# VealFang/PLI-SLAM

Hardware: AMD Instinct MI355X
Metric: stereo frames/sec (ORB+LSD extract+match), 752x480 EuRoC (higher is better)
Workload: dtype u8; 1 GPU; 1xMI355X: 752x480 stereo pairs, extract + stereo Hamming match (BASELINE configs[1] shape, batched); 752x480, 1200 ORB kp (8 levels x1.2) + LSD/LBD (<=100 lines); 256 stereo frames per GPU per step; frames_per_gpu=256, parallelism=frame-batch data parallel, 1 rank(s), gather of result tables to rank 0

## Files before the change

### pli_slam_amd/csrc/kernels.hpp

```cpp
#pragma once
#include "common.hpp"

namespace pli {

struct BlurPlane {
  int w, h, pitchIn, pitchOut;
  int64_t offIn, offOut;
  int tilesX, tileBase;
};
struct BlurJob {
  int nplanes;
  BlurPlane pl[MAX_LEVELS];
  int k[7];
  int radius;
};
struct LbdCoef { float L[21]; float G[63]; };
constexpr int PROJ_K = 64;
__global__ void k_ingest_copy16(const uint8_t* __restrict__ left, const uint8_t* __restrict__ right, int64_t stride, int64_t frameStride, uint8_t* __restrict__ pyr, int64_t pyrBlock, int W16, int H, int pitch, int img0);
__global__ void k_ingest(const uint8_t* __restrict__ left, const uint8_t* __restrict__ right, int64_t stride, int64_t frameStride, uint8_t* __restrict__ pyr, int64_t pyrBlock, int W, int H, int pitch, const float2* __restrict__ mapL, const float2* __restrict__ mapR, int img0);
__global__ void k_resize_level(const uint8_t* __restrict__ srcBase, int64_t srcImgStride, int sw, int sh, int spitch, uint8_t* __restrict__ dstBase, int64_t dstImgStride, int dw, int dh, int dpitch, const int* __restrict__ tab, int img0);
__global__ void k_fast_cells(const DevParams* __restrict__ Pp, const uint8_t* __restrict__ pyr, uint32_t* __restrict__ cellCand, int* __restrict__ cellCount, int img0);
__global__ void k_octree(const DevParams* __restrict__ Pp, const uint32_t* __restrict__ cellCand, const int* __restrict__ cellCount, uint32_t* __restrict__ candAll, unsigned short* __restrict__ nodeOfAll, int* __restrict__ candCount, uint32_t* __restrict__ kpSel, int* __restrict__ kpSelCount, int img0);
__global__ void k_octree_512(const DevParams* __restrict__ Pp, const uint32_t* __restrict__ cellCand, const int* __restrict__ cellCount, uint32_t* __restrict__ candAll, unsigned short* __restrict__ nodeOfAll, int* __restrict__ candCount, uint32_t* __restrict__ kpSel, int* __restrict__ kpSelCount, int img0);
__global__ void k_octree_320(const DevParams* __restrict__ Pp, const uint32_t* __restrict__ cellCand, const int* __restrict__ cellCount, uint32_t* __restrict__ candAll, unsigned short* __restrict__ nodeOfAll, int* __restrict__ candCount, uint32_t* __restrict__ kpSel, int* __restrict__ kpSelCount, int img0);
__global__ void k_octree_w(const DevParams* __restrict__ Pp, const uint32_t* __restrict__ cellCand, const int* __restrict__ cellCount, uint32_t* __restrict__ candAll, unsigned short* __restrict__ nodeOfAll, int* __restrict__ candCount, uint32_t* __restrict__ kpSel, int* __restrict__ kpSelCount, int img0);
__global__ void k_octree_512_w(const DevParams* __restrict__ Pp, const uint32_t* __restrict__ cellCand, const int* __restrict__ cellCount, uint32_t* __restrict__ candAll, unsigned short* __restrict__ nodeOfAll, int* __restrict__ candCount, uint32_t* __restrict__ kpSel, int* __restrict__ kpSelCount, int img0);
__global__ void k_octree_320_w(const DevParams* __restrict__ Pp, const uint32_t* __restrict__ cellCand, const int* __restrict__ cellCount, uint32_t* __restrict__ candAll, unsigned short* __restrict__ nodeOfAll, int* __restrict__ candCount, uint32_t* __restrict__ kpSel, int* __restrict__ kpSelCount, int img0);
__global__ void k_blur(const BlurJob* __restrict__ Jp, const uint8_t* __restrict__ in, int64_t inImgStride, uint8_t* __restrict__ out, int64_t outImgStride, int img0);
__global__ void k_describe(const DevParams* __restrict__ Pp, const uint8_t* __restrict__ pyr, const uint8_t* __restrict__ blur, const uint32_t* __restrict__ kpSel, const int* __restrict__ kpSelCount, uint8_t* __restrict__ table, int64_t recordBytes, int64_t offCounts, int64_t offKp0, int64_t offKp1, int64_t offDesc0, int64_t offDesc1, int img0);
__global__ void k_kp_counts(const DevParams* __restrict__ Pp, const int* __restrict__ kpSelCount, uint8_t* __restrict__ table, int64_t recordBytes, int64_t offCounts, int nimg, int img0);
__global__ void k_lsd_grad(const uint8_t* __restrict__ scaled, int64_t imgStride, int W, int H, int WP, int pitch, int g2Thresh, float4* __restrict__ rec, int* __restrict__ g2o, int2* __restrict__ own, int* __restrict__ maxG2, float* __restrict__ angDbg, int img0, int trigF32);
__global__ void k_lsd_hist(const int* __restrict__ g2a, int npix, int g2Thresh, int nBins, const int* __restrict__ maxG2, unsigned short* __restrict__ chunkHist, int nChunks, int img0, const double* __restrict__ mgAll, const unsigned long long* __restrict__ maxMg, double rho, const RxCtl* __restrict__ onlyUnsettled);
__global__ void k_lsd_scan(const unsigned short* __restrict__ chunkHist, int nChunks, int nBins, int* __restrict__ chunkBase, int* __restrict__ nDefined, int img0, const RxCtl* __restrict__ onlyUnsettled);
__global__ void k_lsd_scatter(const int* __restrict__ g2a, int npix, int g2Thresh, int nBins, const int* __restrict__ maxG2, const int* __restrict__ chunkBase, int nChunks, int* __restrict__ order, int img0, int nimg, const double* __restrict__ mgAll, const unsigned long long* __restrict__ maxMg, double rho, int* __restrict__ rankAll, const int* __restrict__ groupOff, int chunksPerGroup, int nGroups, const RxCtl* __restrict__ onlyUnsettled);
__global__ void k_lsd_scan_part(const unsigned short* __restrict__ chunkHist, int nChunks, int nBins, int chunksPerGroup, int* __restrict__ chunkBase, int* __restrict__ groupOff, int img0, const RxCtl* __restrict__ onlyUnsettled);
__global__ void k_lsd_scan_groups(int nGroups, int nBins, int* __restrict__ groupOff, int* __restrict__ nDefined, int img0, const RxCtl* __restrict__ onlyUnsettled);
__global__ void k_lsd_grow_unsettled(const DevParams* __restrict__ Pp, float4* __restrict__ recAll, const double* __restrict__ mgAll, const int* __restrict__ orderAll, const int* __restrict__ nDefined, uint2* __restrict__ regOverflow, float* __restrict__ segAll, int* __restrict__ nSeg, int maxSeg, int img0, int nimg, RxCtl* __restrict__ ctl);
__global__ void k_lsd_grow(const DevParams* __restrict__ Pp, float4* __restrict__ recAll, const double* __restrict__ mgAll, const int* __restrict__ orderAll, const int* __restrict__ nDefined, uint2* __restrict__ regOverflow, float* __restrict__ segAll, int* __restrict__ nSeg, int maxSeg, int img0, int nimg);
__global__ void k_lsd_grow2(const DevParams* __restrict__ Pp, float4* __restrict__ recAll, const double* __restrict__ mgAll, const int* __restrict__ orderAll, const int* __restrict__ nDefined, uint2* __restrict__ regOverflow, float* __restrict__ segAll, int* __restrict__ nSeg, int maxSeg, int img0, int nimg);
__global__ void k_lsd_grow_spec(const DevParams* __restrict__ Pp, float4* __restrict__ recAll, const double* __restrict__ mgAll, const int* __restrict__ orderAll, const int* __restrict__ nDefined, uint2* __restrict__ regOverflow, float* __restrict__ segAll, int* __restrict__ nSeg, int maxSeg, int img0, int nimg, LsdRectItem* __restrict__ rectAll, double* __restrict__ rectWAll);
__global__ void k_lsd_grow2_spec(const DevParams* __restrict__ Pp, float4* __restrict__ recAll, const double* __restrict__ mgAll, const int* __restrict__ orderAll, const int* __restrict__ nDefined, uint2* __restrict__ regOverflow, float* __restrict__ segAll, int* __restrict__ nSeg, int maxSeg, int img0, int nimg, LsdRectItem* __restrict__ rectAll, double* __restrict__ rectWAll);
__global__ void k_lsd_rect(const DevParams* __restrict__ Pp, const LsdRectItem* __restrict__ rectAll, const uint2* __restrict__ arenaAll, const double* __restrict__ mgAll, const double* __restrict__ rectWAll, const int* __restrict__ nSeg, float* __restrict__ segAll, int maxSeg, int img0);
__global__ void k_keylines(const DevParams* __restrict__ Pp, const float* __restrict__ seg, const int* __restrict__ nSeg, int maxSeg, pli_keyline* __restrict__ tmpKL, uint8_t* __restrict__ table, int64_t recordBytes, int64_t offCounts, int64_t offKl0, int64_t offKl1, int img0);
__global__ void k_sobel(const uint8_t* __restrict__ in, int64_t imgStride, int W, int H, int pitch, short2* __restrict__ dxy, int img0);
__global__ void k_lbd(const DevParams* __restrict__ Pp, const LbdCoef* __restrict__ coef, const short2* __restrict__ dxya, uint8_t* __restrict__ table, int64_t recordBytes, int64_t offCounts, int64_t offKl0, int64_t offKl1, int64_t offLd0, int64_t offLd1, float* __restrict__ dbgFloat, int img0);
__global__ void k_lsd_blur64(const uint8_t* __restrict__ pyr, int64_t pyrBlock, int W, int H, int pitch, const double* __restrict__ kern, int radius, double* __restrict__ out, int64_t outImgStride, int img0);
__global__ void k_lsd_resize64(const double* __restrict__ src, int sw, int sh, double* __restrict__ dst, int dw, int dh, int64_t dstImgStride, const int* __restrict__ tab, int img0);
__global__ void k_lsd_grad64(const double* __restrict__ scaled, int W, int H, int WP, int64_t scaledImgStride, double rho, float4* __restrict__ rec, double* __restrict__ mg, int2* __restrict__ own, unsigned long long* __restrict__ maxMg, float* __restrict__ angDbg, int img0, int flags, int2* __restrict__ hot, float2* __restrict__ cold);
__global__ void k_lsd_front64(const uint8_t* __restrict__ pyr, int64_t pyrBlock, int sw, int sh, int pitch, const double* __restrict__ kern, int radius, const int* __restrict__ tab, int dw, int dh, int dp, double rho, float4* __restrict__ rec, double* __restrict__ mg, int2* __restrict__ own, unsigned long long* __restrict__ maxMg, int img0, int flags, int2* __restrict__ hot, float2* __restrict__ cold);
__global__ void k_rx_guess(const float4* __restrict__ recAll, const int* __restrict__ rankAll, int2* __restrict__ ownAll, int W, int H, float precDeg, int img0);
__global__ void k_rx_diff(RxCtl* __restrict__ ctl, const int2* __restrict__ ownAll, int* __restrict__ tileMinAll, int* __restrict__ tileActAll, int W, int H, int TW, int TH, int t, int img0, const int* __restrict__ tileTouchAll);
__global__ void k_rx_classify(RxCtl* __restrict__ ctl, const int2* __restrict__ ownAll, const int* __restrict__ rankAll, const int2* __restrict__ rgBoxAll, uint8_t* __restrict__ rgCleanAll, const int* __restrict__ tileMinAll, int W, int H, int TW, int TH, int t, int img0);
__global__ void k_rx_seed(RxCtl* __restrict__ ctl, int2* __restrict__ ownAll, const int* __restrict__ rankAll, const float4* __restrict__ recAll, const int* __restrict__ rgSizeAll, const uint8_t* __restrict__ rgCleanAll, RxSeed* __restrict__ smallAll, RxSeed* __restrict__ bigAll, int bigCap, int W, int H, int bigThresh, int t, int img0);
__global__ void k_rx_mark(RxCtl* __restrict__ ctl, const int2* __restrict__ ownAll, const int* __restrict__ rankAll, const int2* __restrict__ rgBoxAll, int* __restrict__ rgDirtyAll, const int* __restrict__ tileMinAll, int* __restrict__ tileActAll, int W, int H, int TW, int TH, int t, int img0, int seedRule, const int* __restrict__ rgLostAll, TxDirtyLists DL);
__global__ void k_rx_seed_sparse(RxCtl* __restrict__ ctl, int2* __restrict__ ownAll, const int* __restrict__ rankAll, const float4* __restrict__ recAll, const int* __restrict__ rgSizeAll, const int* __restrict__ rgDirtyAll, const int* __restrict__ tileActAll, RxSeed* __restrict__ smallAll, RxSeed* __restrict__ bigAll, int bigCap, int W, int H, int TW, int TH, int bigThresh, int t, int img0);
__global__ void k_rx_grow(const DevParams* __restrict__ Pp, RxCtl* __restrict__ ctl, const float4* __restrict__ recAll, int2* __restrict__ ownAll, const RxSeed* __restrict__ smallAll, int* __restrict__ rgSizeAll, int2* __restrict__ rgBoxAll, RxHand* __restrict__ handAll, int handCap, int* __restrict__ arenaAll, int arenaCap, RxRect* __restrict__ rectAll, int rectCap, int img0, int t);
__global__ void k_rx_grow_big(const DevParams* __restrict__ Pp, RxCtl* __restrict__ ctl, const float4* __restrict__ recAll, int2* __restrict__ ownAll, const RxSeed* __restrict__ bigAll, int bigCap, const RxHand* __restrict__ handAll, int handCap, int* __restrict__ rgSizeAll, int2* __restrict__ rgBoxAll, int* __restrict__ arenaAll, int arenaCap, RxRect* __restrict__ rectAll, int rectCap, int img0, int t);
__global__ void k_rx_grow_wave(const DevParams* __restrict__ Pp, RxCtl* __restrict__ ctl, const float4* __restrict__ recAll, int2* __restrict__ ownAll, const RxSeed* __restrict__ bigAll, int bigCap, const RxHand* __restrict__ handAll, int handCap, int* __restrict__ rgSizeAll, int2* __restrict__ rgBoxAll, int* __restrict__ arenaAll, int arenaCap, RxRect* __restrict__ rectAll, int rectCap, int img0, int t);
__global__ void k_rx_rect(const DevParams* __restrict__ Pp, RxCtl* __restrict__ ctl, const float4* __restrict__ recAll, const int* __restrict__ arenaAll, int arenaCap, const RxRect* __restrict__ rectAll, int rectCap, float4* __restrict__ rgSegAll, int img0, const double* __restrict__ mgAll, int rmask, const int2* __restrict__ hotAll, const float2* __restrict__ coldAll);
// ... 60 lines not shown
```

### pli_slam_amd/csrc/line_kernels.hip

```cpp
#include "kernels.hpp"
#include "device_prims.hpp"
#include <type_traits>

namespace pli {

constexpr float LSD_NOTDEF = -1024.f;
constexpr double D_PI = 3.14159265358979323846;
constexpr double D_DEG2RAD = D_PI / 180;
constexpr double D_3_2_PI = (3 * D_PI) / 2;
constexpr double D_2PI = 2 * D_PI;

constexpr int LSD_GRAD_ROWS = 16;

__global__ __launch_bounds__(256) void k_lsd_grad(const uint8_t* __restrict__ scaled, int64_t imgStride, int W, int H,
                                                  int WP ,
                                                  int pitch, int g2Thresh, float4* __restrict__ rec,
                                                  int* __restrict__ g2o, int2* __restrict__ own,
                                                  int* __restrict__ maxG2, float* __restrict__ angDbg, int img0, int trigF32) {
  __shared__ int wmax[4];
  const int img = blockIdx.z + img0;
  const int x = blockIdx.x * 256 + threadIdx.x;
  int m = 0;
  if (x < WP) {
    const int yEnd = min((int)(blockIdx.y + 1) * LSD_GRAD_ROWS, H);
// ... 1329 lines not shown
      }
      if (i < M && rank < nf) {
        pli_keyline kl = tk[i];
        kl.class_id = rank;
        out[rank] = kl;
      }
    }
    if (tid == 0) reinterpret_cast<int*>(rec + offCounts)[2 + eye] = nf;
  } else {
    const int cnt = min(M, P.klCap);
    for (int i = tid; i < cnt; i += 256) out[i] = tk[i];
    if (tid == 0) reinterpret_cast<int*>(rec + offCounts)[2 + eye] = cnt;
  }
}

__global__ __launch_bounds__(256) void k_sobel(const uint8_t* __restrict__ in, int64_t imgStride, int W, int H,
                                               int pitch, short2* __restrict__ dxy, int img0) {
  const int img = blockIdx.z + img0, y = blockIdx.y, x0 = (blockIdx.x * 256 + threadIdx.x) * 4;
  const int lane = threadIdx.x & 63;
  const uint8_t* base = in + (int64_t)img * imgStride;
  const uint8_t* rows[3] = {base + (int64_t)reflect101(y - 1, H) * pitch, base + (int64_t)y * pitch, base + (int64_t)reflect101(y + 1, H) * pitch};
  const bool live = x0 < W;
  int v[3][6];
#pragma unroll
  for (int r = 0; r < 3; ++r) {
    unsigned cur = 0u;
    if (live) cur = *reinterpret_cast<const unsigned*>(rows[r] + x0);
    unsigned prev = (unsigned)__shfl_up((int)cur, 1, 64), next = (unsigned)__shfl_down((int)cur, 1, 64);
    if (lane == 0 && live && x0 >= 4) prev = *reinterpret_cast<const unsigned*>(rows[r] + x0 - 4);
    if (lane == 63 && x0 + 4 < W) next = *reinterpret_cast<const unsigned*>(rows[r] + x0 + 4);
    v[r][1] = cur & 0xFF; v[r][2] = (cur >> 8) & 0xFF; v[r][3] = (cur >> 16) & 0xFF; v[r][4] = cur >> 24;
    v[r][0] = x0 == 0 ? v[r][2] : (int)(prev >> 24);
    v[r][5] = (int)(next & 0xFF);
  }
  if (!live) return;
  if (x0 + 4 >= W) {
#pragma unroll
    for (int r = 0; r < 3; ++r)
#pragma unroll
      for (int k = 1; k < 6; ++k)
        if (x0 + k - 1 >= W) v[r][k] = rows[r][reflect101(min(x0 + k - 1, W), W)];
  }
  short2 o[4];
#pragma unroll
  for (int k = 0; k < 4; ++k) {
    const int gx = (v[0][k + 2] - v[0][k]) + 2 * (v[1][k + 2] - v[1][k]) + (v[2][k + 2] - v[2][k]);
    const int gy = (v[2][k] - v[0][k]) + 2 * (v[2][k + 1] - v[0][k + 1]) + (v[2][k + 2] - v[0][k + 2]);
    o[k] = make_short2((short)gx, (short)gy);
  }
  short2* dst = dxy + (int64_t)img * W * H + (int64_t)y * W + x0;
  if (x0 + 3 < W && (((int64_t)y * W + x0) & 3) == 0 && ((int64_t)W * H & 3) == 0) {
    *reinterpret_cast<int4*>(dst) = make_int4(*reinterpret_cast<int*>(&o[0]), *reinterpret_cast<int*>(&o[1]),
                                              *reinterpret_cast<int*>(&o[2]), *reinterpret_cast<int*>(&o[3]));
  } else {
    for (int k = 0; k < 4 && x0 + k < W; ++k) dst[k] = o[k];
  }
}

__constant__ int c_lbd_comb[32][2] = {
    {0, 1}, {0, 2}, {0, 3}, {0, 4}, {0, 5}, {0, 6}, {1, 2}, {1, 3}, {1, 4}, {1, 5}, {1, 6},
    {2, 3}, {2, 4}, {2, 5}, {2, 6}, {2, 7}, {2, 8}, {3, 4}, {3, 5}, {3, 6}, {3, 7}, {3, 8},
    {4, 5}, {4, 6}, {4, 7}, {4, 8}, {5, 6}, {5, 7}, {5, 8}, {6, 7}, {6, 8}, {7, 8}};


__global__ __launch_bounds__(64) void k_lbd(const DevParams* __restrict__ Pp, const LbdCoef* __restrict__ coef,
                                            const short2* __restrict__ dxya,
                                            uint8_t* __restrict__ table, int64_t recordBytes, int64_t offCounts,
                                            int64_t offKl0, int64_t offKl1, int64_t offLd0, int64_t offLd1,
                                            float* __restrict__ dbgFloat, int img0) {
  __shared__ float rowS[63][4];
// ... 118 lines not shown
```

### pli_slam_amd/csrc/orb_kernels.hip

```cpp
#include "kernels.hpp"
#include <type_traits>
#include "device_prims.hpp"

namespace pli {

__constant__ signed char c_orb_pattern[1024] = {
#include "../../include/pli_orb_pattern.inc"
};

__global__ __launch_bounds__(256) void k_ingest_copy16(const uint8_t* __restrict__ left, const uint8_t* __restrict__ right, int64_t stride,
                                                       int64_t frameStride, uint8_t* __restrict__ pyr, int64_t pyrBlock, int W16, int H,
                                                       int pitch, int img0) {
  const int img = blockIdx.y + img0;
  const uint8_t* src = ((img & 1) ? right : left) + (int64_t)(img >> 1) * frameStride;
  uint8_t* dst = pyr + (int64_t)img * pyrBlock;
  const int n = W16 * H;
  for (int i = blockIdx.x * 256 + threadIdx.x; i < n; i += gridDim.x * 256) {
    const int y = i / W16, x = (i - y * W16) * 16;
    *reinterpret_cast<uint4*>(dst + (int64_t)y * pitch + x) = *reinterpret_cast<const uint4*>(src + (int64_t)y * stride + x);
  }
}

__global__ __launch_bounds__(256) void k_ingest(const uint8_t* __restrict__ left, const uint8_t* __restrict__ right,
                                                int64_t stride, int64_t frameStride, uint8_t* __restrict__ pyr,
// ... 688 lines not shown
        s[0] += kc[k] * v.x; s[1] += kc[k] * v.y; s[2] += kc[k] * v.z; s[3] += kc[k] * v.w;
      }
      uint8_t o[4];
#pragma unroll
      for (int i = 0; i < 4; ++i) {
        int v = (s[i] + (1 << 15)) >> 16;
        o[i] = (uint8_t)(v < 0 ? 0 : (v > 255 ? 255 : v));
      }
      uint8_t* d = dst + (int64_t)(y0 + y) * PL.pitchOut + x0 + 4 * j;
      if (x0 + 4 * j + 3 < PL.w) *reinterpret_cast<uchar4*>(d) = make_uchar4(o[0], o[1], o[2], o[3]);
      else for (int i = 0; i < 4 && x0 + 4 * j + i < PL.w; ++i) d[i] = o[i];
    }
  }
}

__global__ __launch_bounds__(64) void k_describe(const DevParams* __restrict__ Pp, const uint8_t* __restrict__ pyr,
                                                 const uint8_t* __restrict__ blur, const uint32_t* __restrict__ kpSel,
                                                 const int* __restrict__ kpSelCount, uint8_t* __restrict__ table,
                                                 int64_t recordBytes, int64_t offCounts, int64_t offKp0,
                                                 int64_t offKp1, int64_t offDesc0, int64_t offDesc1, int img0) {
  const DevParams& P = *Pp;
  const int img = blockIdx.y + img0, slot = blockIdx.x;
  int lvl = 0;
#pragma unroll 1
  for (int l = 1; l < P.nlevels; ++l)
    if (slot >= P.lv[l].kpBase) lvl = l;
  const LevelGeom& G = P.lv[lvl];
  const int p = slot - G.kpBase;
  const int* cnts = kpSelCount + img * P.nlevels;
  if (p >= cnts[lvl]) return;
  int before = 0, total = 0;
  for (int l = 0; l < P.nlevels; ++l) {
    int c = cnts[l];
    if (l < lvl) before += c;
    total += c;
  }
  const int lane = threadIdx.x;
  uint8_t* rec = table + (int64_t)(img >> 1) * recordBytes;
  const int eye = img & 1;
  (void)offCounts; (void)total;
  const int outIdx = before + p;
  if (outIdx >= P.kpCap) return;
  const uint32_t cv = kpSel[(int64_t)img * P.kpSlotsPerImage + slot];
  const int kx = (int)((cv >> 8) & 0xFFF) + G.minBX, ky = (int)(cv >> 20) + G.minBY;
  const int resp = (int)(cv & 0xFF);
  const uint8_t* im = pyr + (int64_t)img * P.pyrBlock + G.offset;
  __shared__ int s_umax[16];
  if (lane < 16) s_umax[lane] = P.umax[lane];
  __syncthreads();
  int m10 = 0, m01 = 0;
  int val[16];
#pragma unroll
  for (int k = 0; k < 16; ++k) {
    const int i = lane + 64 * k;
    const int r = (i * 2115) >> 16;
    const int v = r - 15, u = (i - r * 31) - 15;
    const int av = v < 0 ? -v : v, au = u < 0 ? -u : u;
    val[k] = 0;
    if (i < 31 * 31 && au <= s_umax[av]) val[k] = im[(int64_t)(ky + v) * G.pitch + kx + u];
  }
#pragma unroll
  for (int k = 0; k < 16; ++k) {
    const int i = lane + 64 * k;
    const int r = (i * 2115) >> 16;
    m10 += ((i - r * 31) - 15) * val[k];
    m01 += (r - 15) * val[k];
  }
  m10 = wave_sum_i32(m10);
  m01 = wave_sum_i32(m01);
  const float angle = fast_atan2_deg((float)m01, (float)m10);
  const float factorPI = (float)(3.14159265358979323846 / 180.f);
  const float ang = __fmul_rn(angle, factorPI);
  float a, b;
  sincos_of_float(ang, (P.parityFlags & PLI_PARITY_TRIG_F32_ORB) != 0, &b, &a);
  const uint8_t* bl = blur + (int64_t)img * P.pyrBlock + G.offset;
  const uint8_t* center = bl + (int64_t)ky * G.pitch + kx;
  unsigned long long words[4];
#pragma unroll
  for (int j = 0; j < 4; ++j) {
    const signed char* pt = c_orb_pattern + 4 * (64 * j + lane);
    float x0 = (float)pt[0], y0 = (float)pt[1], x1 = (float)pt[2], y1 = (float)pt[3];
    int r0 = cv_round_f(__fadd_rn(__fmul_rn(x0, b), __fmul_rn(y0, a)));
    int c0 = cv_round_f(__fsub_rn(__fmul_rn(x0, a), __fmul_rn(y0, b)));
    int r1 = cv_round_f(__fadd_rn(__fmul_rn(x1, b), __fmul_rn(y1, a)));
    int c1 = cv_round_f(__fsub_rn(__fmul_rn(x1, a), __fmul_rn(y1, b)));
    int t0 = center[(int64_t)r0 * G.pitch + c0];
    int t1 = center[(int64_t)r1 * G.pitch + c1];
    words[j] = __ballot(t0 < t1);
  }
  if (lane == 0) {
    pli_keypoint kp;
    kp.x = (float)kx; kp.y = (float)ky;
    if (lvl != 0) { kp.x = __fmul_rn((float)kx, G.scale); kp.y = __fmul_rn((float)ky, G.scale); }
    kp.size = (float)(int)__fmul_rn(31.f, G.scale);
    kp.angle = angle;
    kp.response = (float)resp;
    kp.octave = lvl;
    reinterpret_cast<pli_keypoint*>(rec + (eye ? offKp1 : offKp0))[outIdx] = kp;
    unsigned long long* d = reinterpret_cast<unsigned long long*>(rec + (eye ? offDesc1 : offDesc0) + (int64_t)outIdx * 32);
    d[0] = words[0]; d[1] = words[1]; d[2] = words[2]; d[3] = words[3];
  }
}
// ... 32 lines not shown
```

### pli_slam_amd/csrc/pli_capi.hip

```cpp
#include "kernels.hpp"
#include "scratch_plan.hpp"
#include <cmath>
#include <cfloat>
#include <algorithm>
#include <memory>
#include <limits>
#include <cstdlib>
#include <set>
#include <string>
#include <functional>
#include <mutex>
#include <atomic>
#include <dlfcn.h>

using namespace pli;

#ifdef PLI_DEV
#define DEVENV(name) getenv(name)
#else
static inline const char* pli_no_devenv() { return nullptr; }
#define DEVENV(name) (pli_no_devenv())
#endif

namespace {
// ... 409 lines not shown
  L.off_ldesc[0] = take((int64_t)lc * 32);
  L.off_ldesc[1] = take((int64_t)lc * 32);
  L.off_disp = take((int64_t)lc * 8);
  L.off_le = take((int64_t)lc * 24);
  L.record_bytes = alignUp(o, 256);
}

pli_status allocAll(pli_ctx* c) {
  const DevParams& P = c->hp;
  const int NI = c->NI;
  pli_status st;
#define A(ptr, n) if ((st = c->dalloc(&(ptr), (size_t)(n))) != PLI_OK) return st
  A(c->dP, 1);
  HIPCHK(hipMemcpy(c->dP, &c->hp, sizeof(DevParams), hipMemcpyHostToDevice));
  A(c->pyr, (size_t)P.pyrBlock * NI);
  A(c->blur, (size_t)P.pyrBlock * NI);
  for (int l = 1; l < P.nlevels; ++l) {
    const LevelGeom &S = P.lv[l - 1], &D = P.lv[l];
    std::vector<int> t = buildResizeTab(S.w, S.h, D.w, D.h, 1. / ((double)D.w / S.w), 1. / ((double)D.h / S.h));
    A(c->resizeTab[l], t.size());
    HIPCHK(hipMemcpy(c->resizeTab[l], t.data(), t.size() * 4, hipMemcpyHostToDevice));
  }
  A(c->cellCand, (size_t)NI * P.cellsPerImage * CELL_CAP);
  A(c->cellCount, (size_t)NI * P.cellsPerImage);
  A(c->candAll, (size_t)NI * P.candPerImage);
  A(c->nodeOf, (size_t)NI * P.candPerImage);
  A(c->candCount, (size_t)NI * P.nlevels);
  A(c->kpSel, (size_t)NI * P.kpSlotsPerImage);
  A(c->kpSelCount, (size_t)NI * P.nlevels);
  {
    BlurJob J;
    std::memset(&J, 0, sizeof(J));
    J.nplanes = P.nlevels;
    J.radius = 3;
    gaussKernelFixed8(7, 2.0, J.k);
    int tb = 0;
    for (int l = 0; l < P.nlevels; ++l) {
      BlurPlane& p = J.pl[l];
      p.w = P.lv[l].w; p.h = P.lv[l].h; p.pitchIn = p.pitchOut = P.lv[l].pitch;
      p.offIn = p.offOut = P.lv[l].offset;
      p.tilesX = (p.w + 63) / 64;
      p.tileBase = tb;
      tb += p.tilesX * ((p.h + 31) / 32);
    }
    c->orbTiles = tb;
    A(c->jobOrb, 1);
    HIPCHK(hipMemcpy(c->jobOrb, &J, sizeof(J), hipMemcpyHostToDevice));
    c->tmpPitch = (int)alignUp(P.W, 64);
    c->tmp8Stride = alignUp((int64_t)c->tmpPitch * P.H, 256);
    std::memset(&J, 0, sizeof(J));
    J.nplanes = 1;
    const double sigma = (c->cfg.lsd_scale < 1) ? (c->cfg.lsd_sigma_scale / c->cfg.lsd_scale) : c->cfg.lsd_sigma_scale;
    const unsigned h = (unsigned)std::ceil(sigma * std::sqrt(2 * 3.0 * std::log(10.0)));
    if (h > 3) { g_err = "LSD pre-filter radius > 3 not supported"; return PLI_ERR_INVALID; }
    J.radius = (int)h;
    gaussKernelFixed8(1 + 2 * (int)h, sigma, J.k);
    J.pl[0].w = P.W; J.pl[0].h = P.H; J.pl[0].pitchIn = P.lv[0].pitch; J.pl[0].pitchOut = c->tmpPitch;
    J.pl[0].offIn = P.lv[0].offset; J.pl[0].offOut = 0;
    J.pl[0].tilesX = (P.W + 63) / 64; J.pl[0].tileBase = 0;
    c->l0Tiles = J.pl[0].tilesX * ((P.H + 31) / 32);
    A(c->jobLsd, 1);
    HIPCHK(hipMemcpy(c->jobLsd, &J, sizeof(J), hipMemcpyHostToDevice));
    J.radius = 2;
    std::memset(J.k, 0, sizeof(J.k));
    gaussKernelFixed8(5, 1.0, J.k);
    A(c->jobLbd, 1);
    HIPCHK(hipMemcpy(c->jobLbd, &J, sizeof(J), hipMemcpyHostToDevice));
  }
  A(c->tmp8, (size_t)c->tmp8Stride * NI);
  c->lsdStride = alignUp((int64_t)P.lpitch * P.LH, 256);
  A(c->lsdScaled, (size_t)c->lsdStride * NI);
  if (c->cfg.lsd_scale != 1) {
    std::vector<int> t = buildResizeTab(P.W, P.H, P.LWt, P.LH, 1. / c->cfg.lsd_scale, 1. / c->cfg.lsd_scale);
    A(c->lsdTab, t.size());
    HIPCHK(hipMemcpy(c->lsdTab, t.data(), t.size() * 4, hipMemcpyHostToDevice));
  }
  const size_t npix = (size_t)P.LW * P.LH;
  A(c->rec, npix * NI);
  c->lsdF64 = (c->cfg.parity_flags & PLI_PARITY_LSD_F64) != 0;
  if (c->lsdF64) {
// ... 249 lines not shown
  }
  if (P.cellsPerImage > 0)
    LAUNCH(c, "k_fast_cells", k_fast_cells, dim3(P.cellsPerImage, nimg), dim3(256), 0, c->dP, c->pyr, c->cellCand, c->cellCount, img0);
  {
    int need = 0;
    for (int l = 0; l < P.nlevels; ++l) need = std::max(need, std::max(P.lv[l].nfeatures + 8, 4 * P.lv[l].nIni + 8));
    bool wide = P.nlevels * nimg <= 1024;
    if (const char* e = DEVENV("PLI_OCTREE_WIDE")) wide = atoi(e) != 0;
    const dim3 og(P.nlevels, nimg), ob(wide ? 1024 : 256);
#define OCTREE_LAUNCH(K) LAUNCH(c, "k_octree", K, og, ob, 0, c->dP, c->cellCand, c->cellCount, c->candAll, c->nodeOf, c->candCount, c->kpSel, c->kpSelCount, img0)
    if (need <= 320) { if (wide) OCTREE_LAUNCH(k_octree_320_w); else OCTREE_LAUNCH(k_octree_320); }
    else if (need <= 512) { if (wide) OCTREE_LAUNCH(k_octree_512_w); else OCTREE_LAUNCH(k_octree_512); }
    else { if (wide) OCTREE_LAUNCH(k_octree_w); else OCTREE_LAUNCH(k_octree); }
#undef OCTREE_LAUNCH
  }
  LAUNCH(c, "k_blur_orb", k_blur, dim3(c->orbTiles, nimg), dim3(256), 0, c->jobOrb, c->pyr, P.pyrBlock, c->blur, P.pyrBlock, img0);
  LAUNCH(c, "k_kp_counts", k_kp_counts, dim3((nimg + 63) / 64), dim3(64), 0, c->dP, c->kpSelCount, table, Y.record_bytes,
         Y.off_counts, nimg, img0);
  LAUNCH(c, "k_describe", k_describe, dim3(P.kpSlotsPerImage, nimg), dim3(64), 0, c->dP, c->pyr, c->blur, c->kpSel,
         c->kpSelCount, table, Y.record_bytes, Y.off_counts, Y.off_kp[0], Y.off_kp[1], Y.off_desc[0], Y.off_desc[1], img0);
  return PLI_OK;
}

#define TRL(c, name, ...)                                                      \
  do {                                                                         \
    LAUNCH(c, rxn(name), __VA_ARGS__);                                         \
    if (trace) {                                                               \
      HIPCHK(hipStreamSynchronize((c)->stream));                               \
      std::fprintf(stderr, "[rx] %s done\n", name);                           \
    }                                                                          \
  } while (0)

pli_status runLbdPre(pli_ctx* c, int img0, int nimg) {
  TraceRange range__("pli:lbd blur+sobel");
  const DevParams& P = c->hp;
  LAUNCH(c, "k_blur_lbd", k_blur, dim3(c->l0Tiles, nimg), dim3(256), 0, c->jobLbd, c->pyr, P.pyrBlock, c->tmp8, c->tmp8Stride, img0);
  dim3 g((P.W + 1023) / 1024, P.H, nimg);
  LAUNCH(c, "k_sobel", k_sobel, g, dim3(256), 0, c->tmp8, c->tmp8Stride, P.W, P.H, c->tmpPitch, c->dxy, img0);
  return PLI_OK;
}

pli_status runLines(pli_ctx* c, int img0, int nimg, uint8_t* table) {
  TraceRange range__("pli:line chain");
  const DevParams& P = c->hp;
  const pli_table_layout& Y = c->lay;
  const int npix = P.LW * P.LH;
  const bool sequential = c->lsdMode == 2 || (c->lsdMode == 0 && (nimg >= RX_AUTO_IMAGES || nimg > c->rxImages));
  int2* ownPlane = (sequential || c->lsdMode != 1) ? (int2*)nullptr : c->own;
  const bool lostRule0 = c->lsdMode != 1 && DEVENV("PLI_TX_BOXRULE") == nullptr;
  const bool keyMode = !sequential && c->lsdMode != 1 && c->txKeys && !c->debug && lostRule0 && !DEVENV("PLI_TX_FULL2") &&
                       !DEVENV("PLI_TX_OLDMARK") && !DEVENV("PLI_TX_CELLRULE");
  int packMode = 0;
  if (!sequential && c->lsdMode != 1 && c->lsdF64 && c->mg && lostRule0 && !c->debug && !DEVENV("PLI_TX_FULL2") && !DEVENV("PLI_TX_NOFUSE2") &&
// ... 1911 lines not shown
  for (const std::string& nme : orderNames) {
    std::snprintf(line, sizeof(line), "%s %d %.6f\n", nme.c_str(), acc[nme].first, acc[nme].second);
    s += line;
  }
  if ((int64_t)s.size() + 1 > bytes) { g_err = "report buffer too small"; return PLI_ERR_CAPACITY; }
  std::memcpy(buf, s.c_str(), s.size() + 1);
  return PLI_OK;
}

pli_status pli_debug_enable(pli_ctx* c, int32_t on) {
  CtxGuard guard__(c);
  if (!c) return PLI_ERR_INVALID;
  HIPCHK(hipStreamSynchronize(c->stream));
  if (on && !c->angDbg) {
    pli_status st;
    if ((st = c->dalloc(&c->angDbg, (size_t)c->hp.LW * c->hp.LH * c->NI)) != PLI_OK) return st;
    if ((st = c->dalloc(&c->lbdFloat, (size_t)c->NI * c->hp.klCap * 72)) != PLI_OK) return st;
    if (c->lsdF64 && (st = c->dalloc(&c->scaled64Dbg, (size_t)c->hp.LW * c->hp.LH * c->NI)) != PLI_OK) return st;
  }
  c->debug = on != 0;
  return PLI_OK;
}

pli_status pli_debug_fetch(pli_ctx* c, int32_t image, int32_t what, int32_t arg, void* dst, int64_t dstBytes, int64_t* outBytes) {
  CtxGuard guard__(c);
  if (!c || image < 0 || image >= c->NI || !outBytes) { g_err = "bad argument"; return PLI_ERR_INVALID; }
  HIPCHK(hipSetDevice(c->device));
  HIPCHK(hipStreamSynchronize(c->stream));
  const DevParams& P = c->hp;
  auto need = [&](int64_t n) -> bool { *outBytes = n; return dst && dstBytes >= n; };
  switch (what) {
    case PLI_DBG_PYRAMID_LEVEL:
    case PLI_DBG_BLUR_LEVEL: {
      if (arg < 0 || arg >= P.nlevels) return PLI_ERR_INVALID;
      const LevelGeom& G = P.lv[arg];
      if (!need((int64_t)G.w * G.h)) return dst ? PLI_ERR_CAPACITY : PLI_OK;
      const uint8_t* base = (what == PLI_DBG_PYRAMID_LEVEL ? c->pyr : c->blur) + (int64_t)image * P.pyrBlock + G.offset;
      HIPCHK(hipMemcpy2D(dst, G.w, base, G.pitch, G.w, G.h, hipMemcpyDeviceToHost));
      return PLI_OK;
    }
    case PLI_DBG_FAST_CANDIDATES:
    case PLI_DBG_LEVEL_KEYPOINTS: {
      if (arg < 0 || arg >= P.nlevels) return PLI_ERR_INVALID;
      const LevelGeom& G = P.lv[arg];
      int n = 0;
      const int* cntp = (what == PLI_DBG_FAST_CANDIDATES ? c->candCount : c->kpSelCount) + image * P.nlevels + arg;
      HIPCHK(hipMemcpy(&n, cntp, 4, hipMemcpyDeviceToHost));
      if (!need(4 + (int64_t)n * 12)) return dst ? PLI_ERR_CAPACITY : PLI_OK;
      std::vector<uint32_t> raw(std::max(n, 1));
      const uint32_t* src = what == PLI_DBG_FAST_CANDIDATES ? c->candAll + (int64_t)image * P.candPerImage + G.candBase
// ... 96 lines not shown
    case PLI_DBG_STEREO_SAD: {
      const int frame = image >> 1;
      const int64_t n = (int64_t)P.kpCap * 4;
      if (!need(2 * n)) return dst ? PLI_ERR_CAPACITY : PLI_OK;
      HIPCHK(hipMemcpy(dst, c->sad + (int64_t)frame * P.kpCap, n, hipMemcpyDeviceToHost));
      HIPCHK(hipMemcpy((char*)dst + n, c->bestIdx + (int64_t)frame * P.kpCap, n, hipMemcpyDeviceToHost));
      return PLI_OK;
    }
    default:
      g_err = "unknown debug item";
      return PLI_ERR_INVALID;
  }
}

}
```

Baseline: 6315 stereo frames/s.

## Fuse ORB blur into describe and LBD blur into sobel via LDS tiles

k_describe now stages a window around each keypoint in LDS, blurs it locally with v_dot4 separable passes, and samples the BRIEF pattern from that tile instead of reading a full-image blurred pyramid. k_sobel likewise blurs a tile in shared memory before computing gradients, so the separate k_blur launches and the intermediate blur buffers are dropped. This removes full-image blur passes and their global memory traffic, but the blur work is repeated for overlapping keypoint windows, and each describe block now does more LDS work and syncs.

```diff
diff --git a/pli_slam_amd/csrc/kernels.hpp b/pli_slam_amd/csrc/kernels.hpp
--- a/pli_slam_amd/csrc/kernels.hpp
+++ b/pli_slam_amd/csrc/kernels.hpp
@@ -15,6 +15,24 @@
   int radius;
 };
 struct LbdCoef { float L[21]; float G[63]; };
+
+constexpr signed char ORB_PATTERN_HOST[1024] = {
+#include "../../include/pli_orb_pattern.inc"
+};
+constexpr int orbPatternReach() {
+  int best = 0;
+  for (int i = 0; i < 512; ++i) {
+    const long long x = ORB_PATTERN_HOST[2 * i], y = ORB_PATTERN_HOST[2 * i + 1], r2 = x * x + y * y;
+    int n = 0;
+    while ((long long)(2 * n + 1) * (2 * n + 1) * 10000 <= 4 * r2 * 10002) ++n;
+    best = n > best ? n : best;
+  }
+  return best;
+}
+constexpr int ORB_REACH = orbPatternReach();
+constexpr int ORB_BLUR_R = 3;
+constexpr int ORB_HALF_PATCH = 15;
+constexpr int LBD_BLUR_R = 2;
 constexpr int PROJ_K = 64;
 __global__ void k_ingest_copy16(const uint8_t* __restrict__ left, const uint8_t* __restrict__ right, int64_t stride, int64_t frameStride, uint8_t* __restrict__ pyr, int64_t pyrBlock, int W16, int H, int pitch, int img0);
 __global__ void k_ingest(const uint8_t* __restrict__ left, const uint8_t* __restrict__ right, int64_t stride, int64_t frameStride, uint8_t* __restrict__ pyr, int64_t pyrBlock, int W, int H, int pitch, const float2* __restrict__ mapL, const float2* __restrict__ mapR, int img0);
@@ -27,7 +45,7 @@
 __global__ void k_octree_512_w(const DevParams* __restrict__ Pp, const uint32_t* __restrict__ cellCand, const int* __restrict__ cellCount, uint32_t* __restrict__ candAll, unsigned short* __restrict__ nodeOfAll, int* __restrict__ candCount, uint32_t* __restrict__ kpSel, int* __restrict__ kpSelCount, int img0);
 __global__ void k_octree_320_w(const DevParams* __restrict__ Pp, const uint32_t* __restrict__ cellCand, const int* __restrict__ cellCount, uint32_t* __restrict__ candAll, unsigned short* __restrict__ nodeOfAll, int* __restrict__ candCount, uint32_t* __restrict__ kpSel, int* __restrict__ kpSelCount, int img0);
 __global__ void k_blur(const BlurJob* __restrict__ Jp, const uint8_t* __restrict__ in, int64_t inImgStride, uint8_t* __restrict__ out, int64_t outImgStride, int img0);
-__global__ void k_describe(const DevParams* __restrict__ Pp, const uint8_t* __restrict__ pyr, const uint8_t* __restrict__ blur, const uint32_t* __restrict__ kpSel, const int* __restrict__ kpSelCount, uint8_t* __restrict__ table, int64_t recordBytes, int64_t offCounts, int64_t offKp0, int64_t offKp1, int64_t offDesc0, int64_t offDesc1, int img0);
+__global__ void k_describe(const DevParams* __restrict__ Pp, const uint8_t* __restrict__ pyr, const BlurJob* __restrict__ Jp, const uint32_t* __restrict__ kpSel, const int* __restrict__ kpSelCount, uint8_t* __restrict__ table, int64_t recordBytes, int64_t offCounts, int64_t offKp0, int64_t offKp1, int64_t offDesc0, int64_t offDesc1, int img0);
 __global__ void k_kp_counts(const DevParams* __restrict__ Pp, const int* __restrict__ kpSelCount, uint8_t* __restrict__ table, int64_t recordBytes, int64_t offCounts, int nimg, int img0);
 __global__ void k_lsd_grad(const uint8_t* __restrict__ scaled, int64_t imgStride, int W, int H, int WP, int pitch, int g2Thresh, float4* __restrict__ rec, int* __restrict__ g2o, int2* __restrict__ own, int* __restrict__ maxG2, float* __restrict__ angDbg, int img0, int trigF32);
 __global__ void k_lsd_hist(const int* __restrict__ g2a, int npix, int g2Thresh, int nBins, const int* __restrict__ maxG2, unsigned short* __restrict__ chunkHist, int nChunks, int img0, const double* __restrict__ mgAll, const unsigned long long* __restrict__ maxMg, double rho, const RxCtl* __restrict__ onlyUnsettled);
@@ -42,7 +60,7 @@
 __global__ void k_lsd_grow2_spec(const DevParams* __restrict__ Pp, float4* __restrict__ recAll, const double* __restrict__ mgAll, const int* __restrict__ orderAll, const int* __restrict__ nDefined, uint2* __restrict__ regOverflow, float* __restrict__ segAll, int* __restrict__ nSeg, int maxSeg, int img0, int nimg, LsdRectItem* __restrict__ rectAll, double* __restrict__ rectWAll);
 __global__ void k_lsd_rect(const DevParams* __restrict__ Pp, const LsdRectItem* __restrict__ rectAll, const uint2* __restrict__ arenaAll, const double* __restrict__ mgAll, const double* __restrict__ rectWAll, const int* __restrict__ nSeg, float* __restrict__ segAll, int maxSeg, int img0);
 __global__ void k_keylines(const DevParams* __restrict__ Pp, const float* __restrict__ seg, const int* __restrict__ nSeg, int maxSeg, pli_keyline* __restrict__ tmpKL, uint8_t* __restrict__ table, int64_t recordBytes, int64_t offCounts, int64_t offKl0, int64_t offKl1, int img0);
-__global__ void k_sobel(const uint8_t* __restrict__ in, int64_t imgStride, int W, int H, int pitch, short2* __restrict__ dxy, int img0);
+__global__ void k_sobel(const BlurJob* __restrict__ Jp, const uint8_t* __restrict__ in, int64_t inImgStride, short2* __restrict__ dxy, int img0);
 __global__ void k_lbd(const DevParams* __restrict__ Pp, const LbdCoef* __restrict__ coef, const short2* __restrict__ dxya, uint8_t* __restrict__ table, int64_t recordBytes, int64_t offCounts, int64_t offKl0, int64_t offKl1, int64_t offLd0, int64_t offLd1, float* __restrict__ dbgFloat, int img0);
 __global__ void k_lsd_blur64(const uint8_t* __restrict__ pyr, int64_t pyrBlock, int W, int H, int pitch, const double* __restrict__ kern, int radius, double* __restrict__ out, int64_t outImgStride, int img0);
 __global__ void k_lsd_resize64(const double* __restrict__ src, int sw, int sh, double* __restrict__ dst, int dw, int dh, int64_t dstImgStride, const int* __restrict__ tab, int img0);
diff --git a/pli_slam_amd/csrc/line_kernels.hip b/pli_slam_amd/csrc/line_kernels.hip
--- a/pli_slam_amd/csrc/line_kernels.hip
+++ b/pli_slam_amd/csrc/line_kernels.hip
@@ -1367,46 +1367,127 @@
   }
 }
 
-__global__ __launch_bounds__(256) void k_sobel(const uint8_t* __restrict__ in, int64_t imgStride, int W, int H,
-                                               int pitch, short2* __restrict__ dxy, int img0) {
-  const int img = blockIdx.z + img0, y = blockIdx.y, x0 = (blockIdx.x * 256 + threadIdx.x) * 4;
-  const int lane = threadIdx.x & 63;
-  const uint8_t* base = in + (int64_t)img * imgStride;
-  const uint8_t* rows[3] = {base + (int64_t)reflect101(y - 1, H) * pitch, base + (int64_t)y * pitch, base + (int64_t)reflect101(y + 1, H) * pitch};
-  const bool live = x0 < W;
-  int v[3][6];
-#pragma unroll
-  for (int r = 0; r < 3; ++r) {
-    unsigned cur = 0u;
-    if (live) cur = *reinterpret_cast<const unsigned*>(rows[r] + x0);
-    unsigned prev = (unsigned)__shfl_up((int)cur, 1, 64), next = (unsigned)__shfl_down((int)cur, 1, 64);
-    if (lane == 0 && live && x0 >= 4) prev = *reinterpret_cast<const unsigned*>(rows[r] + x0 - 4);
-    if (lane == 63 && x0 + 4 < W) next = *reinterpret_cast<const unsigned*>(rows[r] + x0 + 4);
-    v[r][1] = cur & 0xFF; v[r][2] = (cur >> 8) & 0xFF; v[r][3] = (cur >> 16) & 0xFF; v[r][4] = cur >> 24;
-    v[r][0] = x0 == 0 ? v[r][2] : (int)(prev >> 24);
-    v[r][5] = (int)(next & 0xFF);
-  }
-  if (!live) return;
-  if (x0 + 4 >= W) {
-#pragma unroll
-    for (int r = 0; r < 3; ++r)
-#pragma unroll
-      for (int k = 1; k < 6; ++k)
-        if (x0 + k - 1 >= W) v[r][k] = rows[r][reflect101(min(x0 + k - 1, W), W)];
-  }
-  short2 o[4];
-#pragma unroll
-  for (int k = 0; k < 4; ++k) {
-    const int gx = (v[0][k + 2] - v[0][k]) + 2 * (v[1][k + 2] - v[1][k]) + (v[2][k + 2] - v[2][k]);
-    const int gy = (v[2][k] - v[0][k]) + 2 * (v[2][k + 1] - v[0][k + 1]) + (v[2][k + 2] - v[0][k + 2]);
-    o[k] = make_short2((short)gx, (short)gy);
-  }
-  short2* dst = dxy + (int64_t)img * W * H + (int64_t)y * W + x0;
-  if (x0 + 3 < W && (((int64_t)y * W + x0) & 3) == 0 && ((int64_t)W * H & 3) == 0) {
-    *reinterpret_cast<int4*>(dst) = make_int4(*reinterpret_cast<int*>(&o[0]), *reinterpret_cast<int*>(&o[1]),
-                                              *reinterpret_cast<int*>(&o[2]), *reinterpret_cast<int*>(&o[3]));
-  } else {
-    for (int k = 0; k < 4 && x0 + k < W; ++k) dst[k] = o[k];
+constexpr int SB_H = LBD_BLUR_R + 1;
+constexpr int SB_SR = 32 + 2 * SB_H;
+constexpr int SB_SD = 18;
+constexpr int SB_BR = 34;
+constexpr int SB_BD = 17;
+static_assert(SB_H <= 4 && LBD_BLUR_R <= 3, "the source tile starts one dword left of the output tile");
+
+__global__ __launch_bounds__(256) void k_sobel(const BlurJob* __restrict__ Jp, const uint8_t* __restrict__ in, int64_t inImgStride,
+                                               short2* __restrict__ dxy, int img0) {
+  __shared__ uint32_t t8[SB_SR * SB_SD + 2];
+  __shared__ __attribute__((aligned(16))) int hs[SB_SR * 4 * SB_BD];
+  __shared__ uint32_t bt[SB_BR * SB_BD];
+  const BlurJob& J = *Jp;
+  const BlurPlane& PL = J.pl[0];
+  const int W = PL.w, H = PL.h;
+  const int img = blockIdx.y + img0;
+  const int ty = blockIdx.x / PL.tilesX, tx = blockIdx.x - ty * PL.tilesX;
+  const int x0 = tx * 64, y0 = ty * 32;
+  constexpr int R = LBD_BLUR_R;
+  const uint8_t* src = in + (int64_t)img * inImgStride + PL.offIn;
+  const int tid = threadIdx.x;
+  int kc[7];
+#pragma unroll
+  for (int k = 0; k < 7; ++k) kc[k] = k <= 2 * R ? J.k[k] : 0;
+  const bool narrow = (kc[0] | kc[1] | kc[2] | kc[3] | kc[4] | kc[5] | kc[6]) < 256;
+  const uint32_t kLo = (uint32_t)kc[0] | ((uint32_t)kc[1] << 8) | ((uint32_t)kc[2] << 16) | ((uint32_t)kc[3] << 24);
+  const uint32_t kHi = (uint32_t)kc[4] | ((uint32_t)kc[5] << 8) | ((uint32_t)kc[6] << 16);
+  for (int i = tid; i < SB_SR * SB_SD; i += 256) {
+    const int y = (int)(((float)i + 0.5f) * (1.0f / SB_SD)), d = i - y * SB_SD;
+    const uint8_t* row = src + (int64_t)reflect101(y0 + y - SB_H, H) * PL.pitchIn;
+    const int px = x0 - 4 + 4 * d;
+    uint32_t v;
+    if (px >= 0 && px + 3 < W) {
+      v = *reinterpret_cast<const uint32_t*>(row + px);
+    } else {
+      v = 0;
+#pragma unroll
+      for (int k = 0; k < 4; ++k) {
+        const int xx = reflect101(min(max(px + k, -SB_H), W - 1 + SB_H), W);
+        v |= (uint32_t)row[xx] << (8 * k);
+      }
+    }
+    t8[i] = v;
+  }
+  if (tid < 2) t8[SB_SR * SB_SD + tid] = 0u;
+  __syncthreads();
+  for (int t = tid; t < SB_SR * SB_BD; t += 256) {
+    const int y = (int)(((float)t + 0.5f) * (1.0f / SB_BD)), j = t - y * SB_BD;
+    const uint32_t* w = &t8[y * SB_SD + j];
+    const uint32_t w0 = w[0], w1 = w[1], w2 = w[2], w3 = w[3];
+    int s[4];
+#pragma unroll
+    for (int i = 0; i < 4; ++i) {
+      constexpr int base = 3 - R;
+      const int off = i + base;
+      const bool q = off >= 4;
+      const uint32_t a0 = q ? w1 : w0, a1 = q ? w2 : w1, a2 = q ? w3 : w2;
+      const uint32_t lo = __builtin_amdgcn_alignbyte(a1, a0, off & 3);
+      const uint32_t hi = __builtin_amdgcn_alignbyte(a2, a1, off & 3);
+      if (narrow) {
+        s[i] = (int)__builtin_amdgcn_udot4(hi, kHi, __builtin_amdgcn_udot4(lo, kLo, 0u, false), false);
+      } else {
+        s[i] = 0;
+#pragma unroll
+        for (int k = 0; k < 4; ++k) s[i] += kc[k] * (int)((lo >> (8 * k)) & 255u);
+#pragma unroll
+        for (int k = 4; k < 7; ++k) s[i] += kc[k] * (int)((hi >> (8 * (k - 4))) & 255u);
+      }
+    }
+    *reinterpret_cast<int4*>(&hs[(y * SB_BD + j) * 4]) = make_int4(s[0], s[1], s[2], s[3]);
+  }
+  __syncthreads();
+  for (int t = tid; t < SB_BR * SB_BD; t += 256) {
+    const int r = (int)(((float)t + 0.5f) * (1.0f / SB_BD)), j = t - r * SB_BD;
+    int s[4] = {0, 0, 0, 0};
+#pragma unroll
+    for (int k = 0; k <= 2 * R; ++k) {
+      const int4 v = *reinterpret_cast<const int4*>(&hs[((r + k) * SB_BD + j) * 4]);
+      s[0] += kc[k] * v.x; s[1] += kc[k] * v.y; s[2] += kc[k] * v.z; s[3] += kc[k] * v.w;
+    }
+    uint32_t o = 0;
+#pragma unroll
+    for (int i = 0; i < 4; ++i) o |= min((uint32_t)(s[i] + (1 << 15)) >> 16, 255u) << (8 * i);
+    bt[t] = o;
+  }
+  __syncthreads();
+  const uint8_t* btb = reinterpret_cast<const uint8_t*>(bt);
+  for (int t = tid; t < 32 * 16; t += 256) {
+    const int yy = t >> 4, j = t & 15;
+    const int y = y0 + yy, x = x0 + 4 * j;
+    if (y >= H || x >= W) continue;
+    const int rr[3] = {reflect101(y - 1, H) - y0 + 1, yy + 1, reflect101(y + 1, H) - y0 + 1};
+    int v[3][6];
+#pragma unroll
+    for (int r = 0; r < 3; ++r) {
+      const uint32_t lo = bt[rr[r] * SB_BD + j], hi = bt[rr[r] * SB_BD + j + 1];
+      v[r][0] = lo & 0xFF; v[r][1] = (lo >> 8) & 0xFF; v[r][2] = (lo >> 16) & 0xFF; v[r][3] = lo >> 24;
+      v[r][4] = hi & 0xFF; v[r][5] = (hi >> 8) & 0xFF;
+      if (x == 0) v[r][0] = v[r][2];
+    }
+    if (x + 4 >= W) {
+#pragma unroll
+      for (int r = 0; r < 3; ++r)
+#pragma unroll
+        for (int k = 1; k < 6; ++k)
+          if (x + k - 1 >= W) v[r][k] = btb[rr[r] * (4 * SB_BD) + reflect101(min(x + k - 1, W), W) - x0 + 1];
+    }
+    short2 o[4];
+#pragma unroll
+    for (int k = 0; k < 4; ++k) {
+      const int gx = (v[0][k + 2] - v[0][k]) + 2 * (v[1][k + 2] - v[1][k]) + (v[2][k + 2] - v[2][k]);
+      const int gy = (v[2][k] - v[0][k]) + 2 * (v[2][k + 1] - v[0][k + 1]) + (v[2][k + 2] - v[0][k + 2]);
+      o[k] = make_short2((short)gx, (short)gy);
+    }
+    short2* dst = dxy + (int64_t)img * W * H + (int64_t)y * W + x;
+    if (x + 3 < W && (((int64_t)y * W + x) & 3) == 0 && ((int64_t)W * H & 3) == 0) {
+      *reinterpret_cast<int4*>(dst) = make_int4(*reinterpret_cast<int*>(&o[0]), *reinterpret_cast<int*>(&o[1]),
+                                                *reinterpret_cast<int*>(&o[2]), *reinterpret_cast<int*>(&o[3]));
+    } else {
+      for (int k = 0; k < 4 && x + k < W; ++k) dst[k] = o[k];
+    }
   }
 }
 
diff --git a/pli_slam_amd/csrc/orb_kernels.hip b/pli_slam_amd/csrc/orb_kernels.hip
--- a/pli_slam_amd/csrc/orb_kernels.hip
+++ b/pli_slam_amd/csrc/orb_kernels.hip
@@ -726,11 +726,26 @@
   }
 }
 
+constexpr int DW_R = (ORB_REACH + ORB_BLUR_R > ORB_HALF_PATCH ? ORB_REACH + ORB_BLUR_R : ORB_HALF_PATCH);
+constexpr int DW_S = 2 * DW_R + 1;
+constexpr int DW_SD = (DW_S + 3 + 3) / 4;
+constexpr int DW_O = DW_R - ORB_REACH - ORB_BLUR_R;
+constexpr int DW_B = 2 * ORB_REACH + 1;
+constexpr int DW_BG = (DW_B + 3) / 4;
+constexpr int DW_BP = 4 * DW_BG;
+constexpr int DW_HR = DW_B + 2 * ORB_BLUR_R;
+static_assert(DW_R >= ORB_REACH + ORB_BLUR_R && DW_R >= ORB_HALF_PATCH, "the staged window covers the blur of every tap and IC_Angle's disc");
+static_assert(DW_O + DW_HR <= DW_S && 3 + DW_O + DW_B - 1 + 2 * ORB_BLUR_R < 4 * DW_SD, "the blur passes stay inside the staged window");
+static_assert(DW_BP % 4 == 0 && ORB_BLUR_R == 3 && DW_O <= 1, "four sums per lane and step; two v_dot4 on the dwords j..j+3 per 7-tap sum");
+
 __global__ __launch_bounds__(64) void k_describe(const DevParams* __restrict__ Pp, const uint8_t* __restrict__ pyr,
-                                                 const uint8_t* __restrict__ blur, const uint32_t* __restrict__ kpSel,
+                                                 const BlurJob* __restrict__ Jp, const uint32_t* __restrict__ kpSel,
                                                  const int* __restrict__ kpSelCount, uint8_t* __restrict__ table,
                                                  int64_t recordBytes, int64_t offCounts, int64_t offKp0,
                                                  int64_t offKp1, int64_t offDesc0, int64_t offDesc1, int img0) {
+  __shared__ uint32_t s_src[DW_S * DW_SD + 2];
+  __shared__ __attribute__((aligned(8))) unsigned short s_hs[DW_HR * DW_BP];
+  __shared__ uint32_t s_bl[DW_B * DW_BG];
   const DevParams& P = *Pp;
   const int img = blockIdx.y + img0, slot = blockIdx.x;
   int lvl = 0;
@@ -759,24 +774,72 @@
   const uint8_t* im = pyr + (int64_t)img * P.pyrBlock + G.offset;
   __shared__ int s_umax[16];
   if (lane < 16) s_umax[lane] = P.umax[lane];
-  __syncthreads();
+  const int wy0 = ky - DW_R, ox = (kx - DW_R) & 3, bx = (kx - DW_R) - ox;
+  for (int i = lane; i < DW_S * DW_SD; i += 64) {
+    const int y = i / DW_SD, d = i - y * DW_SD;
+    const uint8_t* row = im + (int64_t)reflect101(wy0 + y, G.h) * G.pitch;
+    const int px = bx + 4 * d;
+    uint32_t v;
+    if (px >= 0 && px + 3 < G.w) {
+      v = *reinterpret_cast<const uint32_t*>(row + px);
+    } else {
+      v = 0;
+#pragma unroll
+      for (int k = 0; k < 4; ++k) v |= (uint32_t)row[reflect101(px + k, G.w)] << (8 * k);
+    }
+    s_src[i] = v;
+  }
+  if (lane < 2) s_src[DW_S * DW_SD + lane] = 0u;
+  __syncthreads();
+  const uint8_t* srcb = reinterpret_cast<const uint8_t*>(s_src);
   int m10 = 0, m01 = 0;
-  int val[16];
 #pragma unroll
   for (int k = 0; k < 16; ++k) {
     const int i = lane + 64 * k;
     const int r = (i * 2115) >> 16;
     const int v = r - 15, u = (i - r * 31) - 15;
     const int av = v < 0 ? -v : v, au = u < 0 ? -u : u;
-    val[k] = 0;
-    if (i < 31 * 31 && au <= s_umax[av]) val[k] = im[(int64_t)(ky + v) * G.pitch + kx + u];
-  }
-#pragma unroll
-  for (int k = 0; k < 16; ++k) {
-    const int i = lane + 64 * k;
-    const int r = (i * 2115) >> 16;
-    m10 += ((i - r * 31) - 15) * val[k];
-    m01 += (r - 15) * val[k];
+    int val = 0;
+    if (i < 31 * 31 && au <= s_umax[av]) val = srcb[(DW_R + v) * (4 * DW_SD) + ox + DW_R + u];
+    m10 += u * val;
+    m01 += v * val;
+  }
+  const BlurJob& J = *Jp;
+  int kc[7];
+#pragma unroll
+  for (int k = 0; k < 7; ++k) kc[k] = J.k[k];
+  const uint32_t kLo = (uint32_t)kc[0] | ((uint32_t)kc[1] << 8) | ((uint32_t)kc[2] << 16) | ((uint32_t)kc[3] << 24);
+  const uint32_t kHi = (uint32_t)kc[4] | ((uint32_t)kc[5] << 8) | ((uint32_t)kc[6] << 16);
+  for (int t = lane; t < DW_HR * DW_BG; t += 64) {
+    const int y = t / DW_BG, j = t - y * DW_BG;
+    const uint32_t* w = &s_src[(DW_O + y) * DW_SD + j];
+    const uint32_t w0 = w[0], w1 = w[1], w2 = w[2], w3 = w[3];
+    uint32_t s[4];
+#pragma unroll
+    for (int i = 0; i < 4; ++i) {
+      const int off = ox + DW_O + i;
+      const bool q = off >= 4;
+      const uint32_t a0 = q ? w1 : w0, a1 = q ? w2 : w1, a2 = q ? w3 : w2;
+      const uint32_t lo = __builtin_amdgcn_alignbyte(a1, a0, off & 3);
+      const uint32_t hi = __builtin_amdgcn_alignbyte(a2, a1, off & 3);
+      s[i] = __builtin_amdgcn_udot4(hi, kHi, __builtin_amdgcn_udot4(lo, kLo, 0u, false), false);
+    }
+    *reinterpret_cast<uint2*>(&s_hs[y * DW_BP + 4 * j]) = make_uint2(s[0] | (s[1] << 16), s[2] | (s[3] << 16));
+  }
+  __syncthreads();
+  for (int t = lane; t < DW_B * DW_BG; t += 64) {
+    const int y = t / DW_BG, j = t - y * DW_BG;
+    int s[4] = {0, 0, 0, 0};
+#pragma unroll
+    for (int k = 0; k < 7; ++k) {
+      const uint2 v = *reinterpret_cast<const uint2*>(&s_hs[(y + k) * DW_BP + 4 * j]);
+      s[0] += kc[k] * (int)(v.x & 0xFFFFu); s[1] += kc[k] * (int)(v.x >> 16);
+      s[2] += kc[k] * (int)(v.y & 0xFFFFu); s[3] += kc[k] * (int)(v.y >> 16);
+    }
+    uint32_t o = 0;
+#pragma unroll
+    for (int i = 0; i < 4; ++i) o |= min((uint32_t)(s[i] + (1 << 15)) >> 16, 255u) << (8 * i);
+    s_bl[t] = o;
   }
   m10 = wave_sum_i32(m10);
   m01 = wave_sum_i32(m01);
@@ -785,8 +848,8 @@
   const float ang = __fmul_rn(angle, factorPI);
   float a, b;
   sincos_of_float(ang, (P.parityFlags & PLI_PARITY_TRIG_F32_ORB) != 0, &b, &a);
-  const uint8_t* bl = blur + (int64_t)img * P.pyrBlock + G.offset;
-  const uint8_t* center = bl + (int64_t)ky * G.pitch + kx;
+  __syncthreads();
+  const uint8_t* center = reinterpret_cast<const uint8_t*>(s_bl) + ORB_REACH * DW_BP + ORB_REACH;
   unsigned long long words[4];
 #pragma unroll
   for (int j = 0; j < 4; ++j) {
@@ -796,8 +859,8 @@
     int c0 = cv_round_f(__fsub_rn(__fmul_rn(x0, a), __fmul_rn(y0, b)));
     int r1 = cv_round_f(__fadd_rn(__fmul_rn(x1, b), __fmul_rn(y1, a)));
     int c1 = cv_round_f(__fsub_rn(__fmul_rn(x1, a), __fmul_rn(y1, b)));
-    int t0 = center[(int64_t)r0 * G.pitch + c0];
-    int t1 = center[(int64_t)r1 * G.pitch + c1];
+    int t0 = center[r0 * DW_BP + c0];
+    int t1 = center[r1 * DW_BP + c1];
     words[j] = __ballot(t0 < t1);
   }
   if (lane == 0) {
diff --git a/pli_slam_amd/csrc/pli_capi.hip b/pli_slam_amd/csrc/pli_capi.hip
--- a/pli_slam_amd/csrc/pli_capi.hip
+++ b/pli_slam_amd/csrc/pli_capi.hip
@@ -447,7 +447,6 @@
   A(c->dP, 1);
   HIPCHK(hipMemcpy(c->dP, &c->hp, sizeof(DevParams), hipMemcpyHostToDevice));
   A(c->pyr, (size_t)P.pyrBlock * NI);
-  A(c->blur, (size_t)P.pyrBlock * NI);
   for (int l = 1; l < P.nlevels; ++l) {
     const LevelGeom &S = P.lv[l - 1], &D = P.lv[l];
     std::vector<int> t = buildResizeTab(S.w, S.h, D.w, D.h, 1. / ((double)D.w / S.w), 1. / ((double)D.h / S.h));
@@ -465,8 +464,13 @@
     BlurJob J;
     std::memset(&J, 0, sizeof(J));
     J.nplanes = P.nlevels;
-    J.radius = 3;
-    gaussKernelFixed8(7, 2.0, J.k);
+    J.radius = ORB_BLUR_R;
+    gaussKernelFixed8(2 * ORB_BLUR_R + 1, 2.0, J.k);
+    {
+      int ksum = 0, kmax = 0;
+      for (int i = 0; i < 2 * ORB_BLUR_R + 1; ++i) { ksum += J.k[i]; kmax = std::max(kmax, J.k[i]); }
+      if (ksum * 255 > 65535 || kmax > 255) { g_err = "ORB blur coefficients do not fit k_describe's 16-bit sums"; return PLI_ERR_INVALID; }
+    }
     int tb = 0;
     for (int l = 0; l < P.nlevels; ++l) {
       BlurPlane& p = J.pl[l];
@@ -494,9 +498,9 @@
     c->l0Tiles = J.pl[0].tilesX * ((P.H + 31) / 32);
     A(c->jobLsd, 1);
     HIPCHK(hipMemcpy(c->jobLsd, &J, sizeof(J), hipMemcpyHostToDevice));
-    J.radius = 2;
+    J.radius = LBD_BLUR_R;
     std::memset(J.k, 0, sizeof(J.k));
-    gaussKernelFixed8(5, 1.0, J.k);
+    gaussKernelFixed8(2 * LBD_BLUR_R + 1, 1.0, J.k);
     A(c->jobLbd, 1);
     HIPCHK(hipMemcpy(c->jobLbd, &J, sizeof(J), hipMemcpyHostToDevice));
   }
@@ -776,10 +780,11 @@
     else { if (wide) OCTREE_LAUNCH(k_octree_w); else OCTREE_LAUNCH(k_octree); }
 #undef OCTREE_LAUNCH
   }
-  LAUNCH(c, "k_blur_orb", k_blur, dim3(c->orbTiles, nimg), dim3(256), 0, c->jobOrb, c->pyr, P.pyrBlock, c->blur, P.pyrBlock, img0);
+  if (c->debug && c->blur)
+    LAUNCH(c, "k_blur_orb", k_blur, dim3(c->orbTiles, nimg), dim3(256), 0, c->jobOrb, c->pyr, P.pyrBlock, c->blur, P.pyrBlock, img0);
   LAUNCH(c, "k_kp_counts", k_kp_counts, dim3((nimg + 63) / 64), dim3(64), 0, c->dP, c->kpSelCount, table, Y.record_bytes,
          Y.off_counts, nimg, img0);
-  LAUNCH(c, "k_describe", k_describe, dim3(P.kpSlotsPerImage, nimg), dim3(64), 0, c->dP, c->pyr, c->blur, c->kpSel,
+  LAUNCH(c, "k_describe", k_describe, dim3(P.kpSlotsPerImage, nimg), dim3(64), 0, c->dP, c->pyr, c->jobOrb, c->kpSel,
          c->kpSelCount, table, Y.record_bytes, Y.off_counts, Y.off_kp[0], Y.off_kp[1], Y.off_desc[0], Y.off_desc[1], img0);
   return PLI_OK;
 }
@@ -796,9 +801,7 @@
 pli_status runLbdPre(pli_ctx* c, int img0, int nimg) {
   TraceRange range__("pli:lbd blur+sobel");
   const DevParams& P = c->hp;
-  LAUNCH(c, "k_blur_lbd", k_blur, dim3(c->l0Tiles, nimg), dim3(256), 0, c->jobLbd, c->pyr, P.pyrBlock, c->tmp8, c->tmp8Stride, img0);
-  dim3 g((P.W + 1023) / 1024, P.H, nimg);
-  LAUNCH(c, "k_sobel", k_sobel, g, dim3(256), 0, c->tmp8, c->tmp8Stride, P.W, P.H, c->tmpPitch, c->dxy, img0);
+  LAUNCH(c, "k_sobel", k_sobel, dim3(c->l0Tiles, nimg), dim3(256), 0, c->jobLbd, c->pyr, P.pyrBlock, c->dxy, img0);
   return PLI_OK;
 }
 
@@ -2740,6 +2743,7 @@
   HIPCHK(hipStreamSynchronize(c->stream));
   if (on && !c->angDbg) {
     pli_status st;
+    if ((st = c->dalloc(&c->blur, (size_t)c->hp.pyrBlock * c->NI)) != PLI_OK) return st;
     if ((st = c->dalloc(&c->angDbg, (size_t)c->hp.LW * c->hp.LH * c->NI)) != PLI_OK) return st;
     if ((st = c->dalloc(&c->lbdFloat, (size_t)c->NI * c->hp.klCap * 72)) != PLI_OK) return st;
     if (c->lsdF64 && (st = c->dalloc(&c->scaled64Dbg, (size_t)c->hp.LW * c->hp.LH * c->NI)) != PLI_OK) return st;
@@ -2760,6 +2764,7 @@
     case PLI_DBG_BLUR_LEVEL: {
       if (arg < 0 || arg >= P.nlevels) return PLI_ERR_INVALID;
       const LevelGeom& G = P.lv[arg];
+      if (what == PLI_DBG_BLUR_LEVEL && !c->blur) { g_err = "pli_debug_enable was not on during the run"; return PLI_ERR_STATE; }
       if (!need((int64_t)G.w * G.h)) return dst ? PLI_ERR_CAPACITY : PLI_OK;
       const uint8_t* base = (what == PLI_DBG_PYRAMID_LEVEL ? c->pyr : c->blur) + (int64_t)image * P.pyrBlock + G.offset;
       HIPCHK(hipMemcpy2D(dst, G.w, base, G.pitch, G.w, G.h, hipMemcpyDeviceToHost));
@@ -2886,3 +2891,7 @@
 }
 
 }
+
+#ifdef PLI_DEV
+extern "C" int32_t pli_dev_orb_window_reach(void) { return ORB_REACH; }
+#endif
```

Measured after the change: 6413 stereo frames/s, median of 6. +1.6%, better.
